# saurabh260918/Graph-Attention-Network-GATv2-

Measured on AMD Instinct MI355X. Metric: edges/sec (fwd+bwd, 2-layer 8-head GATv2), higher is better.
Workload: dtype f32; 1 GPU; products-shape synthetic power-law graph, 2450000 nodes / 61900000 edges / 100 feat / 47 classes, 2-layer GATv2 heads [8, 8] outdims [8, 8], fp32; launch=eager, parallelism=single GPU, generator=device (csrc/gat_synth.hip), bit-for-bit synth.py

## Files before the change

### graph-attention-network-gatv2-_amd/csrc/gat_dense_kernels.hip

```cpp
#include "gat_internal.h"

#include <algorithm>

#include <cstdlib>

namespace gat {
namespace {

struct MapIdentity {
    __device__ __forceinline__ int64_t operator()(int64_t idx) const { return idx; }
};
struct MapGradW {
    int32_t HD, F, c_base;
    __device__ __forceinline__ int64_t operator()(int64_t idx) const {
        const int32_t c = c_base + (int32_t)idx / F, f = (int32_t)idx % F;
        return (int64_t)(c % HD) * 2 * F + (c / HD) * F + f;
    }
};
template <class MAP>
__global__ __launch_bounds__(1024) void reduce_slabs_kernel(const float* __restrict__ slabs, int32_t nslabs,
                                                           int64_t width, float* __restrict__ out, MAP map) {
    __shared__ float part[16][64];
    const int q = threadIdx.x & 63, sl = threadIdx.x >> 6;
    const int64_t idx = (int64_t)blockIdx.x * 64 + q;
// ... 195 lines not shown
                const int lab_r = A.labels[n0 + r];
                s_dz[r * ldz + c] = lab_r >= 0 ? yt[q] - (c == lab_r ? 1.0f : 0.0f) : 0.0f;
                r += dqC; c += drC;
                if (c >= C) { c -= C; ++r; }
            }
        }
        for (int q = threadIdx.x; q < rows_here * DL; q += 256) s_hl[q] = A.HL[n0 * DL + q];
        __syncthreads();
        {
            int r = threadIdx.x / DL, d = threadIdx.x % DL;
            for (int q = threadIdx.x; q < rows_here * DL; q += 256) {
                float sum = 0.f;
                for (int c = 0; c < C; ++c) sum += s_wo[c * DL + d] * s_dz[r * ldz + c];
                s_gh[q] = sum;
                r += dqD; d += drD;
                if (d >= DL) { d -= DL; ++r; }
            }
        }
#pragma unroll
        for (int p = 0; p < 8; ++p) {
            const int t = threadIdx.x + p * 256;
            if (p < per_thread && t < C * DL) {
                const int c = t / DL, d = t % DL;
                float acc = wacc[p];
                for (int r = 0; r < rows_here; ++r) acc += s_dz[r * ldz + c] * s_hl[r * DL + d];
                wacc[p] = acc;
            }
        }
        __syncthreads();
        if (A.gh_out != nullptr)
            for (int q = threadIdx.x; q < rows_here * DL; q += 256) A.gh_out[(n0 + q / DL) * (A.gh_stride ? A.gh_stride : DL) + q % DL] = s_gh[q];
        if (A.g != nullptr) {
            const float* hp = A.hpre + n0 * hd;
            float* gt = A.g + n0 * hd;
            int r = threadIdx.x / hd, x = threadIdx.x % hd;
            for (int q = threadIdx.x; q < rows_here * hd; q += 256) {
                const int d = x % DL;
                const float hv = A.flat_index ? A.hpre[(n0 + r) * DL + d] : hp[q];
                gt[q] = s_gh[r * DL + d] * (hv > 0.f ? 1.0f : A.slope) * inv_heads;
                r += dqH; x += drH;
                if (x >= hd) { x -= hd; ++r; }
            }
        }
        __syncthreads();
    }
#pragma unroll
    for (int p = 0; p < 8; ++p) {
        const int t = threadIdx.x + p * 256;
        if (p < per_thread && t < C * DL) A.partial[(int64_t)blockIdx.x * C * DL + t] = wacc[p];
    }
}

template <int DL>
__global__ __launch_bounds__(256) void head_backward2_kernel(HeadBwdArgs A, int32_t ldz) {
    constexpr int NB = 128;
    extern __shared__ float lds[];
    const int C = A.C;
    float* s_wo = lds;
    float* s_dz = s_wo + C * DL;
    float* s_hl = s_dz + NB * ldz;
    for (int i = threadIdx.x; i < C * DL; i += 256) s_wo[i] = A.Wo[i];
    const int tid = threadIdx.x;
    const int t2 = tid - 128;
    const int wc = t2 >= 0 ? t2 % C : 0, whalf = t2 >= 0 ? t2 / C : 2;
    float wacc[DL];
#pragma unroll
    for (int d = 0; d < DL; ++d) wacc[d] = 0.f;
    const int64_t ntiles = (A.n_rows + NB - 1) / NB;
    const int dqC = 256 / C, drC = 256 % C;
    for (int64_t tile = blockIdx.x; tile < ntiles; tile += gridDim.x) {
        const int64_t n0 = tile * NB;
        const int rows_here = (int)((A.n_rows - n0 < NB) ? (A.n_rows - n0) : NB);
        __syncthreads();
        {
            const float* yt = A.y + n0 * C;
            int r = tid / C, c = tid % C;
            for (int q = tid; q < rows_here * C; q += 256) {
                const int lab_r = A.labels[n0 + r];
                s_dz[r * ldz + c] = lab_r >= 0 ? yt[q] - (c == lab_r ? 1.0f : 0.0f) : 0.0f;
                r += dqC; c += drC;
                if (c >= C) { c -= C; ++r; }
            }
        }
        for (int q = tid; q < rows_here * DL; q += 256) s_hl[q] = A.HL[n0 * DL + q];
        __syncthreads();
        if (tid < 128) {
            if (tid < rows_here) {
                float acc[DL];
#pragma unroll
                for (int d = 0; d < DL; ++d) acc[d] = 0.f;
                const float* zr = s_dz + tid * ldz;
                for (int c = 0; c < C; ++c) {
                    const float z = zr[c];
#pragma unroll
                    for (int d = 0; d < DL; ++d) acc[d] += s_wo[c * DL + d] * z;
                }
                float* out = A.gh_out + (n0 + tid) * (A.gh_stride ? A.gh_stride : DL);
#pragma unroll
                for (int d = 0; d < DL; ++d) out[d] = acc[d];
            }
        } else if (whalf < 2) {
            const int r0 = whalf * 64, r1 = (r0 + 64 < rows_here) ? r0 + 64 : rows_here;
            for (int r = r0; r < r1; ++r) {
                const float z = s_dz[r * ldz + wc];
#pragma unroll
                for (int d = 0; d < DL; ++d) wacc[d] += z * s_hl[r * DL + d];
            }
        }
    }
    __syncthreads();
    float* s_tmp = s_dz;
    if (whalf < 2) {
#pragma unroll
        for (int d = 0; d < DL; ++d) s_tmp[(whalf * C + wc) * DL + d] = wacc[d];
    }
    __syncthreads();
    for (int i = tid; i < C * DL; i += 256) A.partial[(int64_t)blockIdx.x * C * DL + i] = s_tmp[i] + s_tmp[C * DL + i];
}

template <int DL>
__global__ __launch_bounds__(256) void head_step_kernel(HeadArgs F, HeadBwdArgs A, int32_t ldz) {
    constexpr int NB = 128;
    extern __shared__ float lds[];
    const int C = A.C;
    float* s_wo = lds;
    float* s_dz = s_wo + C * DL;
    float* s_hl = s_dz + NB * ldz;
    __shared__ double s_loss[2];
    __shared__ int32_t s_corr[2];
    for (int i = threadIdx.x; i < C * DL; i += 256) s_wo[i] = A.Wo[i];
    const int tid = threadIdx.x;
    const int t2 = tid - 128;
    const int wc = t2 >= 0 ? t2 % C : 0, whalf = t2 >= 0 ? t2 / C : 2;
    float wacc[DL];
#pragma unroll
    for (int d = 0; d < DL; ++d) wacc[d] = 0.f;
    double loss_acc = 0.0;
    int corr_acc = 0;
    const int64_t ntiles = (A.n_rows + NB - 1) / NB;
    for (int64_t tile = blockIdx.x; tile < ntiles; tile += gridDim.x) {
        const int64_t n0 = tile * NB;
        const int rows_here = (int)((A.n_rows - n0 < NB) ? (A.n_rows - n0) : NB);
        __syncthreads();
        if (tid < rows_here) {
            const int64_t n = n0 + tid;
            float x[DL];
#pragma unroll
            for (int j = 0; j < DL; ++j) { x[j] = A.HL[n * DL + j]; s_hl[tid * DL + j] = x[j]; }
            float* zr = s_dz + tid * ldz;
            float mv = -INFINITY;
            for (int c = 0; c < C; ++c) {
                float acc = 0.f;
#pragma unroll
                for (int j = 0; j < DL; ++j) acc += s_wo[c * DL + j] * x[j];
                zr[c] = acc;
                mv = fmaxf(mv, acc);
            }
            float sum = 0.f;
            for (int c = 0; c < C; ++c) { const float ev = __builtin_amdgcn_exp2f((zr[c] - mv) * 1.4426950408889634f); zr[c] = ev; sum += ev; }
            const double rden = 1.0 / ((double)sum + 1e-8);
            const int lab = A.labels[n];
            float best = -1.f; int pred = 0; float plab = 0.f;
            for (int c = 0; c < C; ++c) {
                const float yv = (float)((double)zr[c] * rden);
                if (c == 0 || yv > best) { best = yv; pred = c; }
                if (c == lab) plab = yv;
                zr[c] = lab >= 0 ? yv - (c == lab ? 1.0f : 0.0f) : 0.0f;
            }
            loss_acc += lab >= 0 ? (double)(-logf(fmaxf(plab, 1e-12f))) : 0.0;
            corr_acc += (lab >= 0 && pred == lab) ? 1 : 0;
        }
        __syncthreads();
        if (tid < 128) {
            if (tid < rows_here) {
                float acc[DL];
#pragma unroll
                for (int d = 0; d < DL; ++d) acc[d] = 0.f;
                const float* zr = s_dz + tid * ldz;
                for (int c = 0; c < C; ++c) {
                    const float z = zr[c];
#pragma unroll
                    for (int d = 0; d < DL; ++d) acc[d] += s_wo[c * DL + d] * z;
                }
                if (A.gh_out != nullptr) {
                    float* out = A.gh_out + (n0 + tid) * (A.gh_stride ? A.gh_stride : DL);
#pragma unroll
                    for (int d = 0; d < DL; ++d) out[d] = acc[d];
                }
            }
        } else if (whalf < 2) {
            const int r0 = whalf * 64, r1 = (r0 + 64 < rows_here) ? r0 + 64 : rows_here;
            for (int r = r0; r < r1; ++r) {
                const float z = s_dz[r * ldz + wc];
#pragma unroll
                for (int d = 0; d < DL; ++d) wacc[d] += z * s_hl[r * DL + d];
            }
        }
    }
    __syncthreads();
    float* s_tmp = s_dz;
    if (whalf < 2) {
#pragma unroll
        for (int d = 0; d < DL; ++d) s_tmp[(whalf * C + wc) * DL + d] = wacc[d];
    }
    for (int off = 32; off > 0; off >>= 1) {
        loss_acc += __shfl_down(loss_acc, off);
        corr_acc += __shfl_down(corr_acc, off);
    }
    if (tid < 128 && (tid & 63) == 0) { s_loss[tid >> 6] = loss_acc; s_corr[tid >> 6] = corr_acc; }
    __syncthreads();
    for (int i = tid; i < C * DL; i += 256) A.partial[(int64_t)blockIdx.x * C * DL + i] = s_tmp[i] + s_tmp[C * DL + i];
    if (tid == 0) {
        F.loss_partial[blockIdx.x] = s_loss[0] + s_loss[1];
        F.correct_partial[blockIdx.x] = s_corr[0] + s_corr[1];
    }
}

__global__ __launch_bounds__(256) void sgd_kernel(float* p, const float* g, float lr, int64_t n) {
    const int64_t i = (int64_t)blockIdx.x * blockDim.x + threadIdx.x;
    if (i < n) p[i] -= lr * g[i];
}
__global__ __launch_bounds__(256) void adam_kernel(float* p, const float* g, float* m, float* v, float lr,
                                                  int64_t n, float b1, float b2, float eps, int32_t t) {
    const int64_t i = (int64_t)blockIdx.x * blockDim.x + threadIdx.x;
    if (i < n) {
        const float gi = g[i];
        const float mi = b1 * m[i] + (1.0f - b1) * gi;
        const float vi = b2 * v[i] + (1.0f - b2) * (gi * gi);
        m[i] = mi; v[i] = vi;
        const float mh = mi / (1.0f - powf(b1, (float)t));
        const float vh = vi / (1.0f - powf(b2, (float)t));
        p[i] -= lr * mh / (sqrtf(vh) + eps);
    }
}
__global__ __launch_bounds__(1024) void sumsq_kernel(const float* __restrict__ g, int64_t n, float* out) {
    __shared__ float part[16];
    float s = 0.f;
    for (int64_t i = threadIdx.x; i < n; i += blockDim.x) s += g[i] * g[i];
    for (int off = 32; off > 0; off >>= 1) s += __shfl_down(s, off);
    if ((threadIdx.x & 63) == 0) part[threadIdx.x >> 6] = s;
    __syncthreads();
    if (threadIdx.x == 0) {
        float t = 0.f;
        for (int w = 0; w < 16; ++w) t += part[w];
        *out = t;
    }
}
__global__ __launch_bounds__(256) void clip_scale_kernel(float* g, int64_t n, const float* sumsq, float thresh) {
    const float norm = sqrtf(*sumsq);
    float scale = 1.0f;
    if (norm > thresh) scale = thresh / (norm + 1e-9f);
    if (!(scale < 1.0f)) return;
    const int64_t i = (int64_t)blockIdx.x * blockDim.x + threadIdx.x;
    if (i < n) g[i] *= scale;
}

template <int V>
__global__ __launch_bounds__(256) void res_backward_kernel(ResBwdArgs A, int32_t LPR, int32_t rpb) {
    __shared__ float red[256 * 4];
    const int HD = A.H * A.D;
    const int t = threadIdx.x;
    const int r_in = t / LPR, cl = t % LPR;
    const float inv_heads = 1.0f / (float)A.H;
    for (int base = 0; base < HD; base += LPR * V) {
        const int c0 = base + cl * V;
        const bool active = r_in < rpb && c0 < HD;
        float sum[V];
// ... 270 lines not shown
    return 0;
}

int launch_reduce_partials_add(const float* partial, int32_t nblocks, int64_t width, float* out, hipStream_t s) {
    if (width <= 0) return 0;
    if (reduce_batch_push(partial, nblocks, width, out, 0, 0, 0)) return 0;
    hipLaunchKernelGGL((reduce_slabs_kernel<MapIdentity>), dim3((unsigned)((width + 63) / 64)), dim3(1024), 0, s,
                       partial, nblocks, width, out, MapIdentity{});
    GAT_HIP(hipGetLastError());
    return 0;
}

static int head_tile(int32_t C, int32_t DL, int32_t extra_per_row, int32_t* NB, int32_t* ldz) {
    const int l = (C % 2 == 0) ? C + 1 : C;
    int64_t budget = 60 * 1024 / 4 - (int64_t)C * DL;
    int nb = 256;
    while (nb >= 32 && (int64_t)nb * (l + extra_per_row) > budget) nb >>= 1;
    if (nb < 32) return fail(GAT_E_UNSUPPORTED, "output head: num_classes*D_last too large for the LDS tile");
    *NB = nb; *ldz = l;
    return 0;
}
int head_blocks(int64_t n_rows) {
    static const int per = [] { const char* e = choice_env("GAT_HEAD_NODES"); const int v = e ? atoi(e) : 0; return v == 256 ? 256 : 128; }();
    const int64_t b = (n_rows + per - 1) / per;
    return (int)(b < 1 ? 1 : (b > 2048 ? 2048 : b));
}
int launch_head_forward(const HeadArgs& a, hipStream_t s) {
    int32_t NB, ldz;
    const int dlp = a.DL <= 8 ? 8 : (a.DL <= 16 ? 16 : (a.DL <= 32 ? 32 : (a.DL <= 64 ? 64 : 0)));
    GAT_TRY(head_tile(a.C, dlp ? dlp : a.DL, 0, &NB, &ldz));
    int blocks = head_blocks(a.n_rows);
    const size_t lds = ((size_t)a.C * (dlp ? dlp : a.DL) + (size_t)NB * ldz) * sizeof(float);
    {
        const void* fn = dlp == 8 ? (const void*)head_forward_kernel<8> : dlp == 16 ? (const void*)head_forward_kernel<16>
                       : dlp == 32 ? (const void*)head_forward_kernel<32> : dlp == 64 ? (const void*)head_forward_kernel<64>
                                                                                      : (const void*)head_forward_kernel<0>;
        const int64_t res = resident_blocks(fn, lds);
        if (res < blocks) blocks = (int)res;
    }
    switch (dlp) {
        case 8: hipLaunchKernelGGL(head_forward_kernel<8>, dim3(blocks), dim3(256), lds, s, a, NB, ldz); break;
        case 16: hipLaunchKernelGGL(head_forward_kernel<16>, dim3(blocks), dim3(256), lds, s, a, NB, ldz); break;
        case 32: hipLaunchKernelGGL(head_forward_kernel<32>, dim3(blocks), dim3(256), lds, s, a, NB, ldz); break;
        case 64: hipLaunchKernelGGL(head_forward_kernel<64>, dim3(blocks), dim3(256), lds, s, a, NB, ldz); break;
        default: hipLaunchKernelGGL(head_forward_kernel<0>, dim3(blocks), dim3(256), lds, s, a, NB, ldz); break;
    }
    GAT_HIP(hipGetLastError());
    hipLaunchKernelGGL(head_finalize_kernel, dim3(1), dim3(64), 0, s, a.loss_partial, a.correct_partial, blocks,
                       a.loss_out, a.correct_out);
    GAT_HIP(hipGetLastError());
    return 0;
}
bool head_step_supported(const HeadBwdArgs& b) {
    return b.g == nullptr && b.gh_out != nullptr && b.C <= 64 && (b.DL == 4 || b.DL == 8 || b.DL == 16);
}
int launch_head_step(const HeadArgs& f, const HeadBwdArgs& b, hipStream_t s) {
    HeadBwdArgs probe = b;
    if (probe.gh_out == nullptr) probe.gh_out = reinterpret_cast<float*>(1);
    if (!head_step_supported(probe)) return fail(GAT_E_UNSUPPORTED, "head_step: shape outside the fused kernel");
    const int ldz = (b.C % 2 == 0) ? b.C + 1 : b.C;
    const size_t lds = ((size_t)b.C * b.DL + (size_t)128 * (ldz + b.DL)) * sizeof(float);
    int blocks = std::min(head_blocks(b.n_rows), head_bwd_blocks(b.n_rows, b.C, b.DL));
    const void* fn = b.DL == 4 ? (const void*)head_step_kernel<4> : b.DL == 8 ? (const void*)head_step_kernel<8>
                                                                                : (const void*)head_step_kernel<16>;
    const int64_t res = resident_blocks(fn, lds);
    if (res < blocks) blocks = (int)res;
    if (blocks < 1) blocks = 1;
    if (b.DL == 4) hipLaunchKernelGGL(head_step_kernel<4>, dim3(blocks), dim3(256), lds, s, f, b, ldz);
    else if (b.DL == 8) hipLaunchKernelGGL(head_step_kernel<8>, dim3(blocks), dim3(256), lds, s, f, b, ldz);
    else hipLaunchKernelGGL(head_step_kernel<16>, dim3(blocks), dim3(256), lds, s, f, b, ldz);
    GAT_HIP(hipGetLastError());
    if (!reduce_batch_finalize(f.loss_partial, f.correct_partial, blocks, f.loss_out, f.correct_out)) {
        hipLaunchKernelGGL(head_finalize_kernel, dim3(1), dim3(64), 0, s, f.loss_partial, f.correct_partial, blocks,
                           f.loss_out, f.correct_out);
        GAT_HIP(hipGetLastError());
    }
    return launch_reduce_partials_add(b.partial, blocks, (int64_t)b.C * b.DL, b.gradWo, s);
}
int launch_pack_result(const float* loss, const int32_t* correct, float* dst3, hipStream_t s) {
    hipLaunchKernelGGL(pack_result_kernel, dim3(1), dim3(64), 0, s, loss, correct, dst3);
    GAT_HIP(hipGetLastError());
    return 0;
}
int head_bwd_blocks(int64_t n_rows, int32_t C, int32_t DL) {
    (void)C; (void)DL;
    const int64_t b = (n_rows + 127) / 128;
    return (int)(b < 1 ? 1 : (b > 1024 ? 1024 : b));
}
int launch_head_backward(const HeadBwdArgs& a, hipStream_t s) {
    if (a.g == nullptr && a.gh_out != nullptr && a.C <= 64 && (a.DL == 4 || a.DL == 8 || a.DL == 16)) {
        const int ldz = (a.C % 2 == 0) ? a.C + 1 : a.C;
        const size_t lds = ((size_t)a.C * a.DL + (size_t)128 * (ldz + a.DL)) * sizeof(float);
        int blocks = (int)std::min<int64_t>((a.n_rows + 127) / 128, 1024);
        const void* fn = a.DL == 4 ? (const void*)head_backward2_kernel<4> : a.DL == 8 ? (const void*)head_backward2_kernel<8>
                                                                                        : (const void*)head_backward2_kernel<16>;
        const int64_t res = resident_blocks(fn, lds);
        if (res < blocks) blocks = (int)res;
        if (blocks < 1) blocks = 1;
        if (a.DL == 4) hipLaunchKernelGGL(head_backward2_kernel<4>, dim3(blocks), dim3(256), lds, s, a, ldz);
        else if (a.DL == 8) hipLaunchKernelGGL(head_backward2_kernel<8>, dim3(blocks), dim3(256), lds, s, a, ldz);
        else hipLaunchKernelGGL(head_backward2_kernel<16>, dim3(blocks), dim3(256), lds, s, a, ldz);
        GAT_HIP(hipGetLastError());
        return launch_reduce_partials_add(a.partial, blocks, (int64_t)a.C * a.DL, a.gradWo, s);
    }
    int32_t NB, ldz;
    GAT_TRY(head_tile(a.C, a.DL, 2 * a.DL, &NB, &ldz));
    const int per_thread = (a.C * a.DL + 255) / 256;
    if (per_thread > 8) return fail(GAT_E_UNSUPPORTED, "output head: num_classes*D_last > 2048");
    int blocks = head_bwd_blocks(a.n_rows, a.C, a.DL);
    const size_t lds = ((size_t)a.C * a.DL + (size_t)NB * (ldz + 2 * a.DL)) * sizeof(float);
    {
        const int64_t res = resident_blocks((const void*)head_backward_kernel, lds);
        if (res < blocks) blocks = (int)res;
    }
    hipLaunchKernelGGL(head_backward_kernel, dim3(blocks), dim3(256), lds, s, a, NB, ldz, per_thread);
    GAT_HIP(hipGetLastError());
    return launch_reduce_partials_add(a.partial, blocks, (int64_t)a.C * a.DL, a.gradWo, s);
}

__global__ __launch_bounds__(256) void apply_mask_kernel(const int32_t* __restrict__ labels, const uint8_t* __restrict__ mask,
                                                         int32_t* __restrict__ eff, int64_t n) {
    const int64_t stride = (int64_t)gridDim.x * blockDim.x;
    for (int64_t i = (int64_t)blockIdx.x * blockDim.x + threadIdx.x; i < n; i += stride)
        eff[i] = (mask == nullptr || mask[i]) ? labels[i] : ~labels[i];
}
int launch_apply_mask(const int32_t* labels, const uint8_t* mask, int32_t* eff, int64_t n, hipStream_t s) {
    if (n <= 0) return 0;
    hipLaunchKernelGGL(apply_mask_kernel, dim3((unsigned)std::min<int64_t>((n + 255) / 256, 4096)), dim3(256), 0, s, labels, mask, eff, n);
    GAT_HIP(hipGetLastError());
    return 0;
}
__global__ __launch_bounds__(256) void eval_mask_kernel(const float* __restrict__ y, const int32_t* __restrict__ labels,
                                                        const uint8_t* __restrict__ mask, int64_t n, int32_t C,
                                                        double* __restrict__ part_loss, int32_t* __restrict__ part_cnt) {
    __shared__ double s_l[256];
    __shared__ int32_t s_c[256], s_n[256];
    double l = 0.0; int32_t cr = 0, nn = 0;
    for (int64_t i = (int64_t)blockIdx.x * 256 + threadIdx.x; i < n; i += (int64_t)gridDim.x * 256) {
        if (!mask[i]) continue;
        const float* yr = y + i * C;
        const int lab = labels[i];
        float best = -1.f; int pred = 0;
        for (int c = 0; c < C; ++c) if (c == 0 || yr[c] > best) { best = yr[c]; pred = c; }
        l += (double)(-logf(fmaxf(yr[lab], 1e-12f)));
        cr += pred == lab; ++nn;
    }
    s_l[threadIdx.x] = l; s_c[threadIdx.x] = cr; s_n[threadIdx.x] = nn;
    __syncthreads();
    for (int off = 128; off > 0; off >>= 1) {
        if (threadIdx.x < off) { s_l[threadIdx.x] += s_l[threadIdx.x + off]; s_c[threadIdx.x] += s_c[threadIdx.x + off]; s_n[threadIdx.x] += s_n[threadIdx.x + off]; }
        __syncthreads();
    }
    if (threadIdx.x == 0) { part_loss[blockIdx.x] = s_l[0]; part_cnt[2 * blockIdx.x] = s_c[0]; part_cnt[2 * blockIdx.x + 1] = s_n[0]; }
}
int launch_eval_mask(const float* y, const int32_t* labels, const uint8_t* mask, int64_t n, int32_t C, double* part_loss,
                     int32_t* part_cnt, int32_t blocks, hipStream_t s) {
// ... 50 lines not shown
```

### graph-attention-network-gatv2-_amd/csrc/gat_gemm_kernels.hip

```cpp
#include "gat_internal.h"

#include <cstdlib>
#include <map>
#include <mutex>
#include <utility>

namespace gat {
namespace {

typedef float v16f __attribute__((ext_vector_type(16)));

struct ASrcRows {
    const float* X; int32_t ld;
    __device__ __forceinline__ float4 load4(int64_t i, int k) const {
        return *reinterpret_cast<const float4*>(X + i * ld + k);
    }
    __device__ __forceinline__ float load1(int64_t i, int k) const { return X[i * ld + k]; }
};
struct ASrcGcat {
    const float* gPL; const float* gPR; int32_t HD;
    __device__ __forceinline__ float4 load4(int64_t i, int k) const {
        return k < HD ? *reinterpret_cast<const float4*>(gPL + i * HD + k)
                      : *reinterpret_cast<const float4*>(gPR + i * HD + (k - HD));
    }
// ... 42 lines not shown
                PL[i * HD + j] = v;
            }
        } else {
            PR[i * HD + (j - HD)] = v;
        }
    }
};
struct EpiGradX {
    static constexpr bool kTwoPhase = true;
    float* out; const float* hpre_prev; int32_t ld; float slope;
    __device__ __forceinline__ float pre(int64_t i, int j) const { return hpre_prev[i * ld + j]; }
    __device__ __forceinline__ void apply(int64_t i, int j, float v, float hv) const {
        out[i * ld + j] = v * (hv > 0.f ? 1.0f : slope);
    }
    __device__ __forceinline__ void operator()(int64_t i, int j, float v) const { apply(i, j, v, pre(i, j)); }
};

struct EpiStore {
    static constexpr bool kTwoPhase = false;
    float* out; int32_t ld;
    __device__ __forceinline__ float pre(int64_t, int) const { return 0.f; }
    __device__ __forceinline__ void apply(int64_t i, int j, float v, float) const { out[i * ld + j] = v; }
    __device__ __forceinline__ void operator()(int64_t i, int j, float v) const { out[i * ld + j] = v; }
};

struct EpiAccum {
    static constexpr bool kTwoPhase = true;
    float* out; int32_t ld;
    __device__ __forceinline__ float pre(int64_t i, int j) const { return out[i * ld + j]; }
    __device__ __forceinline__ void apply(int64_t i, int j, float v, float old) const { out[i * ld + j] = old + v; }
    __device__ __forceinline__ void operator()(int64_t i, int j, float v) const { apply(i, j, v, pre(i, j)); }
};

constexpr int kKC = 128;

}

int64_t resident_blocks(const void* fn, size_t dyn_lds, int threads) {
    static std::mutex mu;
    static std::map<std::pair<const void*, size_t>, int64_t> cache;
    std::lock_guard<std::mutex> lock(mu);
    const auto key = std::make_pair(fn, dyn_lds);
    auto it = cache.find(key);
    if (it != cache.end()) return it->second;
    int per_cu = 0, dev = 0, cus = 256;
    if (hipOccupancyMaxActiveBlocksPerMultiprocessor(&per_cu, fn, threads, dyn_lds) != hipSuccess || per_cu < 1) per_cu = 1;
    if (per_cu > 8) per_cu = 8;
    (void)hipGetDevice(&dev);
    (void)hipDeviceGetAttribute(&cus, hipDeviceAttributeMultiprocessorCount, dev);
    (void)hipGetLastError();
    return cache[key] = (int64_t)per_cu * (cus > 0 ? cus : 256);
}

static void allow_big_lds(const void* fn) {
    static std::mutex mu;
    static std::map<std::pair<const void*, int>, bool> done;
    int dev = 0;
    (void)hipGetDevice(&dev);
    std::lock_guard<std::mutex> lock(mu);
    bool& d = done[std::make_pair(fn, dev)];
    if (!d) { (void)hipFuncSetAttribute(fn, hipFuncAttributeMaxDynamicSharedMemorySize, 160 * 1024); (void)hipGetLastError(); d = true; }
}

namespace {

template <int NT, bool VEC4, class AS, class BS, class EP>
__global__ __launch_bounds__(256) void rowgemm_kernel(AS as, BS bs, EP ep, int64_t M, int32_t N, int32_t K,
                                                      int32_t kc_lds) {
    constexpr int NW = NT * 32;
    extern __shared__ float Bsh[];
    const int lane = threadIdx.x & 63, wave = threadIdx.x >> 6;
    const int li = lane & 31, half = lane >> 5;
    const int n0 = blockIdx.y * NW;
    const int64_t ntiles = (M + 127) / 128;
    bool b_loaded = false;
    for (int64_t tile = blockIdx.x; tile < ntiles; tile += gridDim.x) {
        const int64_t row = tile * 128 + wave * 32 + li;
        const bool rvalid = row < M;
        v16f acc[NT];
#pragma unroll
        for (int nt = 0; nt < NT; ++nt)
#pragma unroll
            for (int r = 0; r < 16; ++r) acc[nt][r] = 0.f;
        for (int k0 = 0; k0 < K; k0 += kKC) {
            const int kc = (K - k0 < kKC) ? (K - k0) : kKC;
            const int kc8 = (kc + 7) & ~7;
            if (K > kKC || !b_loaded) {
                __syncthreads();
                if constexpr (BS::kAlongK) {
                    for (int idx = threadIdx.x; idx < kc8 * NW; idx += 256) {
                        const int kk = idx % kc8, j = idx / kc8;
                        Bsh[kk * NW + j] = (kk < kc && n0 + j < N) ? bs.at(k0 + kk, n0 + j) : 0.f;
                    }
                } else {
                    for (int idx = threadIdx.x; idx < kc8 * NW; idx += 256) {
                        const int kk = idx / NW, j = idx % NW;
                        Bsh[kk * NW + j] = (kk < kc && n0 + j < N) ? bs.at(k0 + kk, n0 + j) : 0.f;
                    }
                }
                b_loaded = true;
                __syncthreads();
            }
            float4 af[kKC / 8];
#pragma unroll
            for (int st = 0; st < kKC / 8; ++st) {
                const int kk = st * 8 + 4 * half;
                af[st] = make_float4(0.f, 0.f, 0.f, 0.f);
// ... 965 lines not shown
```

### graph-attention-network-gatv2-_amd/csrc/gat_internal.h

```cpp
#pragma once
#include <hip/hip_runtime.h>
#include <cstdint>
#include <cstdio>
#include <string>
#include <vector>

#include "gatv2_abi.h"

namespace gat {

constexpr int kWave = 64;

void set_error(const std::string& msg);
int fail(int code, const std::string& msg);
const char* choice_env(const char* name);

#define GAT_HIP(expr)                                                                     \
    do {                                                                                  \
        hipError_t e__ = (expr);                                                          \
        if (e__ != hipSuccess)                                                            \
            return ::gat::fail((int)e__, std::string(#expr) + ": " + hipGetErrorString(e__)); \
    } while (0)

#define GAT_TRY(expr)                 \
// ... 204 lines not shown
int launch_gpl_pull(const SourceIndex& ix, const PullArgs& p, hipStream_t s);

int launch_csr_to_coo(const int32_t* row_ptr, const int32_t* col_idx, int32_t* src, int32_t* dst,
                      int64_t n_rows, int64_t n_edges, int64_t table_row0, hipStream_t s);

struct Comm {
    int world = 1, rank = 0;
    virtual ~Comm();
    virtual int all_gather(float* table, int64_t slice, hipStream_t s) = 0;
    virtual int all_gather_part(float* table, int64_t slice, int64_t off, int64_t cnt, hipStream_t s) = 0;
    virtual int reduce_scatter(float* table, int64_t slice, hipStream_t s) = 0;
    virtual int reduce_scatter_bf16(float* table, int64_t slice, hipStream_t s) = 0;
    virtual int all_reduce(float* buf, int64_t n, hipStream_t s) = 0;
    virtual int exchange_rows(const float* sendbuf, const int64_t* cnt_send, float* recvbuf, const int64_t* cnt_recv, int64_t rf, hipStream_t s) = 0;
};
struct HaloPlan {
    int world = 0, rank = 0;
    int64_t max_rows = 0;
    std::vector<int64_t> need_cnt, send_cnt;
    int64_t n_need = 0, n_send = 0, buf_rows = 0;
    int32_t* need_rows = nullptr;
    int32_t* send_rows = nullptr;
    int32_t *arr_ptr = nullptr, *arr_split = nullptr, *arr_pos = nullptr;
    float *sendbuf = nullptr, *recvbuf = nullptr;
    double referenced_fraction = 1.0;
};
int halo_build(Comm* comm, const int32_t* d_col_idx, int64_t n_edges, int64_t n_table, int32_t hd_max, HaloPlan* out, hipStream_t s);
int halo_forward(Comm* comm, const HaloPlan& h, float* table, int64_t rf, hipStream_t s);
int halo_backward(Comm* comm, const HaloPlan& h, float* gPL, int64_t rf, hipStream_t s);
void halo_free(HaloPlan* h);
int comm_unique_id(void* id_out);
int comm_create_rccl(int world, int rank, const void* id_bytes, Comm** out);
int comm_create_host(int world, int rank, const char* shm_name, int64_t bytes_per_rank, Comm** out);

int launch_pack_result(const float* loss, const int32_t* correct, float* dst3, hipStream_t s);
struct ReduceJob { const float* slabs; float* out; int64_t width; int32_t nslabs, HD, F, c_base, block0; };
struct ReduceBatch {
    ReduceJob jobs[8]; int32_t n, blocks;
    const float* loss; const int32_t* correct; float* dst3; float* dst3_host;
    const double* fin_loss; const int32_t* fin_corr; int32_t fin_n; float* fin_loss_out; int32_t* fin_corr_out;
};
void reduce_batch_begin();
void reduce_batch_abort();
void reduce_batch_pack(const float* loss, const int32_t* correct, float* dst3, float* dst3_host);
bool reduce_batch_finalize(const double* loss_partial, const int32_t* correct_partial, int32_t nblocks, float* loss_out, int32_t* correct_out);
int reduce_batch_flush(hipStream_t s);
int launch_reduce_partials_add(const float* partial, int32_t nblocks, int64_t width, float* out,
                               hipStream_t s);

int launch_reduce_gradw(const float* slabs, int32_t ksplit, int32_t HD, int32_t F, int32_t c_base, int32_t M,
                        float* gradW, hipStream_t s);

int64_t resident_blocks(const void* fn, size_t dyn_lds, int threads = 256);

int launch_transpose_eh_to_he(const float* src_eh, float* dst_he, int64_t E, int32_t H, hipStream_t s);
int launch_transpose_he_to_eh(const float* src_he, float* dst_eh, int64_t E, int32_t H, hipStream_t s);
int launch_transpose_nh_to_hn(const float* src_nh, float* dst_hn, int64_t N, int32_t H, hipStream_t s);

enum : int32_t { kPartBoth = 0, kPartLeft = 1, kPartRight = 2 };
int64_t project_scratch_floats(int64_t n_rows, int32_t F, int32_t HD, int32_t part);
int launch_project(const float* X, const float* W, float* PL_rows, float* PR, int64_t n_rows,
                   int32_t F, int32_t HD, int32_t part, bool pl_bf16, float* scratch, int64_t scratch_floats, hipStream_t s, int32_t ldx = 0);
int64_t grad_w_scratch_floats(int64_t n_rows, int32_t F, int32_t HD);
int launch_grad_w(const float* gPL_rows, const float* gPR, const float* X, float* gradW,
                  float* scratch, int64_t n_rows, int32_t F, int32_t HD, int32_t part, hipStream_t s, int32_t ldx = 0);
int launch_grad_x(const float* gPL_rows, const float* gPR, const float* W, const float* hpre_prev,
                  float* gprev, int64_t n_rows, int32_t F, int32_t HD, float slope, hipStream_t s);

int launch_project_res(const float* X, const float* Wres, float* R, int64_t n_rows, int32_t F, int32_t HD, hipStream_t s, int32_t ldx = 0);
int launch_grad_wres(const float* G, const float* X, float* gradWres, float* scratch, int64_t n_rows, int32_t F, int32_t HD,
                     hipStream_t s, int32_t ldx = 0);
int launch_grad_x_res(const float* G, const float* Wres, float* gx, int64_t n_rows, int32_t F, int32_t HD, hipStream_t s);
struct ResBwdArgs {
    const float* hpre; const float* g; const float* gh; const float* res; const float* bias;
    float* G; float* agg; float* partial;
    int64_t n_rows;
    int32_t H, D, gh_stride, g_raw, blocks;
    float slope;
};
constexpr int kResPartialRows = 1024;
int res_backward_blocks(int64_t n_rows, int32_t HD);
int launch_res_backward(const ResBwdArgs& a, hipStream_t s);

struct NormBwdArgs {
    ResBwdArgs r;
    const float* gamma; const float* beta;
    float* part_gamma; float* part_beta;
    float eps;
};
int norm_backward_blocks(int64_t n_rows, int32_t HD);
int launch_norm_backward(const NormBwdArgs& a, hipStream_t s);

struct HeadArgs {
    const float* Wo;
    const float* HL;
    const int32_t* labels;
    float* y;
    double* loss_partial;
    int32_t* correct_partial;
    float* loss_out;
    int32_t* correct_out;
    int64_t n_rows;
    int32_t C, DL;
};
int head_blocks(int64_t n_rows);
int launch_head_forward(const HeadArgs& a, hipStream_t s);
// ... 77 lines not shown
```

Before: 2.970 billion edges/s.

## Restructure output-head kernels with 256-row tiles, register softmax, and virtual-block partials

Reworks the fused head step and head backward kernels. Tiles grow to 256 rows and all 256 threads now do both the per-row gradient and the Wo-gradient accumulation. Partials are written per fixed virtual block (capped at 1024) instead of per launched block, so the reduction width no longer depends on occupancy. In the step kernel, logits and softmax stay in registers with the class count padded to a compile-time size, HL rows are prefetched with float4 loads for the next tile, and gradient outputs are stored as float4. The cost is more LDS per block (it may need the big-LDS opt-in), more frequent flush barriers, an alignment requirement for the fused path, and more template instantiations.

```diff
diff --git a/graph-attention-network-gatv2-_amd/csrc/gat_dense_kernels.hip b/graph-attention-network-gatv2-_amd/csrc/gat_dense_kernels.hip
--- a/graph-attention-network-gatv2-_amd/csrc/gat_dense_kernels.hip
+++ b/graph-attention-network-gatv2-_amd/csrc/gat_dense_kernels.hip
@@ -271,23 +271,57 @@
 }
 
 template <int DL>
-__global__ __launch_bounds__(256) void head_backward2_kernel(HeadBwdArgs A, int32_t ldz) {
-    constexpr int NB = 128;
-    extern __shared__ float lds[];
+__device__ __forceinline__ void head_wo_tile(const float* s_dz, int ldz, const float* s_hl, int wc, int r0, int r1, float (&wacc)[DL]) {
+    for (int r = r0; r < r1; ++r) {
+        const float zv = s_dz[r * ldz + wc];
+        float h[DL];
+#pragma unroll
+        for (int v = 0; v < DL / 4; ++v) {
+            const float4 q = reinterpret_cast<const float4*>(s_hl + r * DL)[v];
+            h[4 * v] = q.x; h[4 * v + 1] = q.y; h[4 * v + 2] = q.z; h[4 * v + 3] = q.w;
+        }
+#pragma unroll
+        for (int d = 0; d < DL; ++d) wacc[d] = __builtin_fmaf(zv, h[d], wacc[d]);
+    }
+}
+template <int DL>
+__device__ __forceinline__ void head_wo_flush(float* s_tmp, int C, int G, bool owner, float (&wacc)[DL], float* __restrict__ out) {
+    const int tid = threadIdx.x;
+    __syncthreads();
+    if (owner) {
+#pragma unroll
+        for (int d = 0; d < DL; ++d) { s_tmp[tid * DL + d] = wacc[d]; wacc[d] = 0.f; }
+    }
+    __syncthreads();
+    for (int i = tid; i < C * DL; i += 256) {
+        float t = s_tmp[i];
+        for (int g = 1; g < G; ++g) t += s_tmp[g * C * DL + i];
+        out[i] = t;
+    }
+}
+__device__ __forceinline__ void head_next_tile(int64_t ntiles, int VB, int64_t& vb, int64_t& tile) {
+    tile += VB;
+    if (tile >= ntiles) { vb += gridDim.x; tile = vb; }
+}
+
+template <int DL>
+__global__ __launch_bounds__(256) void head_backward2_kernel(HeadBwdArgs A, int32_t ldz, int32_t G, int32_t RPG, int32_t VB) {
+    constexpr int NB = 256;
+    extern __shared__ float4 lds_waves[];
     const int C = A.C;
-    float* s_wo = lds;
+    float* s_hl = reinterpret_cast<float*>(lds_waves);
+    float* s_wo = s_hl + NB * DL;
     float* s_dz = s_wo + C * DL;
-    float* s_hl = s_dz + NB * ldz;
-    for (int i = threadIdx.x; i < C * DL; i += 256) s_wo[i] = A.Wo[i];
     const int tid = threadIdx.x;
-    const int t2 = tid - 128;
-    const int wc = t2 >= 0 ? t2 % C : 0, whalf = t2 >= 0 ? t2 / C : 2;
+    for (int i = tid; i < C * DL; i += 256) s_wo[i] = A.Wo[i];
+    const int wc = tid % C, wg = tid / C;
     float wacc[DL];
 #pragma unroll
     for (int d = 0; d < DL; ++d) wacc[d] = 0.f;
     const int64_t ntiles = (A.n_rows + NB - 1) / NB;
     const int dqC = 256 / C, drC = 256 % C;
-    for (int64_t tile = blockIdx.x; tile < ntiles; tile += gridDim.x) {
+    int64_t vb = blockIdx.x, tile = vb;
+    while (vb < VB) {
         const int64_t n0 = tile * NB;
         const int rows_here = (int)((A.n_rows - n0 < NB) ? (A.n_rows - n0) : NB);
         __syncthreads();
@@ -303,135 +337,143 @@
         }
         for (int q = tid; q < rows_here * DL; q += 256) s_hl[q] = A.HL[n0 * DL + q];
         __syncthreads();
-        if (tid < 128) {
-            if (tid < rows_here) {
-                float acc[DL];
-#pragma unroll
-                for (int d = 0; d < DL; ++d) acc[d] = 0.f;
-                const float* zr = s_dz + tid * ldz;
-                for (int c = 0; c < C; ++c) {
-                    const float z = zr[c];
-#pragma unroll
-                    for (int d = 0; d < DL; ++d) acc[d] += s_wo[c * DL + d] * z;
-                }
-                float* out = A.gh_out + (n0 + tid) * (A.gh_stride ? A.gh_stride : DL);
-#pragma unroll
-                for (int d = 0; d < DL; ++d) out[d] = acc[d];
-            }
-        } else if (whalf < 2) {
-            const int r0 = whalf * 64, r1 = (r0 + 64 < rows_here) ? r0 + 64 : rows_here;
-            for (int r = r0; r < r1; ++r) {
-                const float z = s_dz[r * ldz + wc];
-#pragma unroll
-                for (int d = 0; d < DL; ++d) wacc[d] += z * s_hl[r * DL + d];
-            }
-        }
-    }
-    __syncthreads();
-    float* s_tmp = s_dz;
-    if (whalf < 2) {
-#pragma unroll
-        for (int d = 0; d < DL; ++d) s_tmp[(whalf * C + wc) * DL + d] = wacc[d];
-    }
-    __syncthreads();
-    for (int i = tid; i < C * DL; i += 256) A.partial[(int64_t)blockIdx.x * C * DL + i] = s_tmp[i] + s_tmp[C * DL + i];
+        if (tid < rows_here) {
+            float acc[DL];
+#pragma unroll
+            for (int d = 0; d < DL; ++d) acc[d] = 0.f;
+            const float* zr = s_dz + tid * ldz;
+            for (int c = 0; c < C; ++c) {
+                const float z = zr[c];
+#pragma unroll
+                for (int d = 0; d < DL; ++d) acc[d] = __builtin_fmaf(s_wo[c * DL + d], z, acc[d]);
+            }
+            float* out = A.gh_out + (n0 + tid) * (A.gh_stride ? A.gh_stride : DL);
+#pragma unroll
+            for (int d = 0; d < DL; ++d) out[d] = acc[d];
+        }
+        if (wg < G) head_wo_tile<DL>(s_dz, ldz, s_hl, wc, wg * RPG, (wg * RPG + RPG < rows_here) ? wg * RPG + RPG : rows_here, wacc);
+        const int64_t done = vb;
+        head_next_tile(ntiles, VB, vb, tile);
+        if (vb != done) head_wo_flush<DL>(s_dz, C, G, wg < G, wacc, A.partial + done * C * DL);
+    }
 }
 
 template <int DL>
-__global__ __launch_bounds__(256) void head_step_kernel(HeadArgs F, HeadBwdArgs A, int32_t ldz) {
-    constexpr int NB = 128;
-    extern __shared__ float lds[];
+__device__ __forceinline__ float head_logit(const float* w, const float* x, float z0) {
+    constexpr int NF = DL == 16 ? 4 : 0;
+    float acc = z0;
+#pragma unroll
+    for (int j = 0; j < NF; ++j) acc = __builtin_fmaf(w[j], x[j], acc);
+    {
+#pragma clang fp contract(off)
+#pragma unroll
+        for (int j = NF; j < DL; ++j) acc = acc + w[j] * x[j];
+    }
+    return acc;
+}
+template <int V>
+__device__ __forceinline__ void head_row_load(const float* p, float4 (&x)[V]) {
+#pragma unroll
+    for (int v = 0; v < V; ++v) x[v] = reinterpret_cast<const float4*>(p)[v];
+}
+
+template <int DL, int CP>
+__global__ __launch_bounds__(256) void head_step_kernel(HeadArgs F, HeadBwdArgs A, int32_t G, int32_t RPG, int32_t VB) {
+    constexpr int NB = 256, V = DL / 4, ldz = CP + 1;
+    extern __shared__ float4 lds_waves[];
     const int C = A.C;
-    float* s_wo = lds;
-    float* s_dz = s_wo + C * DL;
-    float* s_hl = s_dz + NB * ldz;
-    __shared__ double s_loss[2];
-    __shared__ int32_t s_corr[2];
-    for (int i = threadIdx.x; i < C * DL; i += 256) s_wo[i] = A.Wo[i];
+    float* s_hl = reinterpret_cast<float*>(lds_waves);
+    float* s_wo = s_hl + NB * DL;
+    float* s_z0 = s_wo + CP * DL;
+    float* s_dz = s_z0 + CP;
+    __shared__ double s_loss[4];
+    __shared__ int32_t s_corr[4];
     const int tid = threadIdx.x;
-    const int t2 = tid - 128;
-    const int wc = t2 >= 0 ? t2 % C : 0, whalf = t2 >= 0 ? t2 / C : 2;
+    for (int i = tid; i < CP * DL; i += 256) s_wo[i] = i < C * DL ? A.Wo[i] : 0.f;
+    if (tid < CP) s_z0[tid] = tid < C ? 0.f : -INFINITY;
+    const int wc = tid % C, wg = tid / C;
     float wacc[DL];
 #pragma unroll
     for (int d = 0; d < DL; ++d) wacc[d] = 0.f;
     double loss_acc = 0.0;
     int corr_acc = 0;
     const int64_t ntiles = (A.n_rows + NB - 1) / NB;
-    for (int64_t tile = blockIdx.x; tile < ntiles; tile += gridDim.x) {
+    const int gstride = A.gh_stride ? A.gh_stride : DL;
+    float4 xn[V] = {};
+    int labn = -1;
+    int64_t vb = blockIdx.x, tile = vb;
+    if (vb < VB && tile * NB + tid < A.n_rows) {
+        head_row_load<V>(A.HL + (tile * NB + tid) * DL, xn);
+        labn = A.labels[tile * NB + tid];
+    }
+    while (vb < VB) {
         const int64_t n0 = tile * NB;
         const int rows_here = (int)((A.n_rows - n0 < NB) ? (A.n_rows - n0) : NB);
+        float x[DL];
+#pragma unroll
+        for (int v = 0; v < V; ++v) { x[4 * v] = xn[v].x; x[4 * v + 1] = xn[v].y; x[4 * v + 2] = xn[v].z; x[4 * v + 3] = xn[v].w; }
+        const int lab = labn;
+        const int64_t done = vb;
+        head_next_tile(ntiles, VB, vb, tile);
+        if (vb < VB && tile * NB + tid < A.n_rows) {
+            head_row_load<V>(A.HL + (tile * NB + tid) * DL, xn);
+            labn = A.labels[tile * NB + tid];
+        }
         __syncthreads();
         if (tid < rows_here) {
-            const int64_t n = n0 + tid;
-            float x[DL];
-#pragma unroll
-            for (int j = 0; j < DL; ++j) { x[j] = A.HL[n * DL + j]; s_hl[tid * DL + j] = x[j]; }
+#pragma unroll
+            for (int v = 0; v < V; ++v) reinterpret_cast<float4*>(s_hl + tid * DL)[v] = make_float4(x[4 * v], x[4 * v + 1], x[4 * v + 2], x[4 * v + 3]);
+            float z[CP];
+            float mv = -INFINITY;
+#pragma unroll
+            for (int c = 0; c < CP; ++c) {
+                const float acc = head_logit<DL>(s_wo + c * DL, x, s_z0[c]);
+                z[c] = acc;
+                mv = fmaxf(mv, acc);
+            }
+            float sum = 0.f;
+#pragma unroll
+            for (int c = 0; c < CP; ++c) { const float ev = __builtin_amdgcn_exp2f((z[c] - mv) * 1.4426950408889634f); z[c] = ev; sum += ev; }
+            const double rden = 1.0 / ((double)sum + 1e-8);
+            float best = -1.f; int pred = 0; float plab = 0.f;
             float* zr = s_dz + tid * ldz;
-            float mv = -INFINITY;
-            for (int c = 0; c < C; ++c) {
-                float acc = 0.f;
-#pragma unroll
-                for (int j = 0; j < DL; ++j) acc += s_wo[c * DL + j] * x[j];
-                zr[c] = acc;
-                mv = fmaxf(mv, acc);
-            }
-            float sum = 0.f;
-            for (int c = 0; c < C; ++c) { const float ev = __builtin_amdgcn_exp2f((zr[c] - mv) * 1.4426950408889634f); zr[c] = ev; sum += ev; }
-            const double rden = 1.0 / ((double)sum + 1e-8);
-            const int lab = A.labels[n];
-            float best = -1.f; int pred = 0; float plab = 0.f;
-            for (int c = 0; c < C; ++c) {
-                const float yv = (float)((double)zr[c] * rden);
+#pragma unroll
+            for (int c = 0; c < CP; ++c) {
+                const float yv = (float)((double)z[c] * rden);
                 if (c == 0 || yv > best) { best = yv; pred = c; }
                 if (c == lab) plab = yv;
-                zr[c] = lab >= 0 ? yv - (c == lab ? 1.0f : 0.0f) : 0.0f;
+                z[c] = lab >= 0 ? yv - (c == lab ? 1.0f : 0.0f) : 0.0f;
+                zr[c] = z[c];
             }
             loss_acc += lab >= 0 ? (double)(-logf(fmaxf(plab, 1e-12f))) : 0.0;
             corr_acc += (lab >= 0 && pred == lab) ? 1 : 0;
+            if (A.gh_out != nullptr) {
+                float acc[DL];
+#pragma unroll
+                for (int d = 0; d < DL; ++d) acc[d] = 0.f;
+#pragma unroll
+                for (int c = 0; c < CP; ++c) {
+#pragma unroll
+                    for (int d = 0; d < DL; ++d) acc[d] = __builtin_fmaf(s_wo[c * DL + d], z[c], acc[d]);
+                }
+                float4* out = reinterpret_cast<float4*>(A.gh_out + (n0 + tid) * gstride);
+#pragma unroll
+                for (int v = 0; v < V; ++v) out[v] = make_float4(acc[4 * v], acc[4 * v + 1], acc[4 * v + 2], acc[4 * v + 3]);
+            }
         }
         __syncthreads();
-        if (tid < 128) {
-            if (tid < rows_here) {
-                float acc[DL];
-#pragma unroll
-                for (int d = 0; d < DL; ++d) acc[d] = 0.f;
-                const float* zr = s_dz + tid * ldz;
-                for (int c = 0; c < C; ++c) {
-                    const float z = zr[c];
-#pragma unroll
-                    for (int d = 0; d < DL; ++d) acc[d] += s_wo[c * DL + d] * z;
-                }
-                if (A.gh_out != nullptr) {
-                    float* out = A.gh_out + (n0 + tid) * (A.gh_stride ? A.gh_stride : DL);
-#pragma unroll
-                    for (int d = 0; d < DL; ++d) out[d] = acc[d];
-                }
-            }
-        } else if (whalf < 2) {
-            const int r0 = whalf * 64, r1 = (r0 + 64 < rows_here) ? r0 + 64 : rows_here;
-            for (int r = r0; r < r1; ++r) {
-                const float z = s_dz[r * ldz + wc];
-#pragma unroll
-                for (int d = 0; d < DL; ++d) wacc[d] += z * s_hl[r * DL + d];
-            }
-        }
-    }
-    __syncthreads();
-    float* s_tmp = s_dz;
-    if (whalf < 2) {
-#pragma unroll
-        for (int d = 0; d < DL; ++d) s_tmp[(whalf * C + wc) * DL + d] = wacc[d];
+        if (wg < G) head_wo_tile<DL>(s_dz, ldz, s_hl, wc, wg * RPG, (wg * RPG + RPG < rows_here) ? wg * RPG + RPG : rows_here, wacc);
+        if (vb != done) head_wo_flush<DL>(s_dz, C, G, wg < G, wacc, A.partial + done * C * DL);
     }
     for (int off = 32; off > 0; off >>= 1) {
         loss_acc += __shfl_down(loss_acc, off);
         corr_acc += __shfl_down(corr_acc, off);
     }
-    if (tid < 128 && (tid & 63) == 0) { s_loss[tid >> 6] = loss_acc; s_corr[tid >> 6] = corr_acc; }
+    if ((tid & 63) == 0) { s_loss[tid >> 6] = loss_acc; s_corr[tid >> 6] = corr_acc; }
     __syncthreads();
-    for (int i = tid; i < C * DL; i += 256) A.partial[(int64_t)blockIdx.x * C * DL + i] = s_tmp[i] + s_tmp[C * DL + i];
     if (tid == 0) {
-        F.loss_partial[blockIdx.x] = s_loss[0] + s_loss[1];
-        F.correct_partial[blockIdx.x] = s_corr[0] + s_corr[1];
+        F.loss_partial[blockIdx.x] = (s_loss[0] + s_loss[1]) + (s_loss[2] + s_loss[3]);
+        F.correct_partial[blockIdx.x] = (s_corr[0] + s_corr[1]) + (s_corr[2] + s_corr[3]);
     }
 }
 
@@ -808,30 +850,52 @@
     return 0;
 }
 bool head_step_supported(const HeadBwdArgs& b) {
-    return b.g == nullptr && b.gh_out != nullptr && b.C <= 64 && (b.DL == 4 || b.DL == 8 || b.DL == 16);
+    const bool vec16 = ((reinterpret_cast<uintptr_t>(b.HL) | reinterpret_cast<uintptr_t>(b.gh_out)) & 15) == 0 && b.gh_stride % 4 == 0;
+    return b.g == nullptr && b.gh_out != nullptr && b.C <= 64 && (b.DL == 4 || b.DL == 8 || b.DL == 16) && vec16;
+}
+struct HeadTree { int32_t VB, G, RPG; };
+static HeadTree head_tree(int64_t n_rows, int32_t C) {
+    const int64_t tiles = (n_rows + 255) / 256;
+    HeadTree t;
+    t.VB = (int32_t)(tiles < 1 ? 1 : (tiles > 1024 ? 1024 : tiles));
+    t.G = 256 / C;
+    t.RPG = (256 + t.G - 1) / t.G;
+    return t;
+}
+template <int DL, int CP>
+static int launch_head_step_cp(const HeadArgs& f, const HeadBwdArgs& b, const HeadTree& t, int* blocks_out, hipStream_t s) {
+    const size_t lds = ((size_t)256 * DL + (size_t)CP * DL + CP + (size_t)256 * std::max(CP + 1, DL)) * sizeof(float);
+    const void* fn = (const void*)head_step_kernel<DL, CP>;
+    if (lds > 64 * 1024) allow_big_lds(fn);
+    int64_t blocks = std::min<int64_t>(t.VB, resident_blocks(fn, lds));
+    if (blocks < 1) blocks = 1;
+    hipLaunchKernelGGL((head_step_kernel<DL, CP>), dim3((unsigned)blocks), dim3(256), lds, s, f, b, t.G, t.RPG, t.VB);
+    GAT_HIP(hipGetLastError());
+    *blocks_out = (int)blocks;
+    return 0;
+}
+template <int DL>
+static int launch_head_step_dl(const HeadArgs& f, const HeadBwdArgs& b, const HeadTree& t, int* blocks_out, hipStream_t s) {
+    if (b.C <= 16) return launch_head_step_cp<DL, 16>(f, b, t, blocks_out, s);
+    if (b.C <= 32) return launch_head_step_cp<DL, 32>(f, b, t, blocks_out, s);
+    if (b.C <= 48) return launch_head_step_cp<DL, 48>(f, b, t, blocks_out, s);
+    return launch_head_step_cp<DL, 64>(f, b, t, blocks_out, s);
 }
 int launch_head_step(const HeadArgs& f, const HeadBwdArgs& b, hipStream_t s) {
     HeadBwdArgs probe = b;
-    if (probe.gh_out == nullptr) probe.gh_out = reinterpret_cast<float*>(1);
+    if (probe.gh_out == nullptr) probe.gh_out = const_cast<float*>(b.HL);
     if (!head_step_supported(probe)) return fail(GAT_E_UNSUPPORTED, "head_step: shape outside the fused kernel");
-    const int ldz = (b.C % 2 == 0) ? b.C + 1 : b.C;
-    const size_t lds = ((size_t)b.C * b.DL + (size_t)128 * (ldz + b.DL)) * sizeof(float);
-    int blocks = std::min(head_blocks(b.n_rows), head_bwd_blocks(b.n_rows, b.C, b.DL));
-    const void* fn = b.DL == 4 ? (const void*)head_step_kernel<4> : b.DL == 8 ? (const void*)head_step_kernel<8>
-                                                                                : (const void*)head_step_kernel<16>;
-    const int64_t res = resident_blocks(fn, lds);
-    if (res < blocks) blocks = (int)res;
-    if (blocks < 1) blocks = 1;
-    if (b.DL == 4) hipLaunchKernelGGL(head_step_kernel<4>, dim3(blocks), dim3(256), lds, s, f, b, ldz);
-    else if (b.DL == 8) hipLaunchKernelGGL(head_step_kernel<8>, dim3(blocks), dim3(256), lds, s, f, b, ldz);
-    else hipLaunchKernelGGL(head_step_kernel<16>, dim3(blocks), dim3(256), lds, s, f, b, ldz);
-    GAT_HIP(hipGetLastError());
+    const HeadTree t = head_tree(b.n_rows, b.C);
+    int blocks = 0;
+    if (b.DL == 4) GAT_TRY((launch_head_step_dl<4>(f, b, t, &blocks, s)));
+    else if (b.DL == 8) GAT_TRY((launch_head_step_dl<8>(f, b, t, &blocks, s)));
+    else GAT_TRY((launch_head_step_dl<16>(f, b, t, &blocks, s)));
     if (!reduce_batch_finalize(f.loss_partial, f.correct_partial, blocks, f.loss_out, f.correct_out)) {
         hipLaunchKernelGGL(head_finalize_kernel, dim3(1), dim3(64), 0, s, f.loss_partial, f.correct_partial, blocks,
                            f.loss_out, f.correct_out);
         GAT_HIP(hipGetLastError());
     }
-    return launch_reduce_partials_add(b.partial, blocks, (int64_t)b.C * b.DL, b.gradWo, s);
+    return launch_reduce_partials_add(b.partial, t.VB, (int64_t)b.C * b.DL, b.gradWo, s);
 }
 int launch_pack_result(const float* loss, const int32_t* correct, float* dst3, hipStream_t s) {
     hipLaunchKernelGGL(pack_result_kernel, dim3(1), dim3(64), 0, s, loss, correct, dst3);
@@ -845,19 +909,19 @@
 }
 int launch_head_backward(const HeadBwdArgs& a, hipStream_t s) {
     if (a.g == nullptr && a.gh_out != nullptr && a.C <= 64 && (a.DL == 4 || a.DL == 8 || a.DL == 16)) {
+        const HeadTree t = head_tree(a.n_rows, a.C);
         const int ldz = (a.C % 2 == 0) ? a.C + 1 : a.C;
-        const size_t lds = ((size_t)a.C * a.DL + (size_t)128 * (ldz + a.DL)) * sizeof(float);
-        int blocks = (int)std::min<int64_t>((a.n_rows + 127) / 128, 1024);
+        const size_t lds = ((size_t)256 * a.DL + (size_t)a.C * a.DL + (size_t)256 * std::max(ldz, a.DL)) * sizeof(float);
         const void* fn = a.DL == 4 ? (const void*)head_backward2_kernel<4> : a.DL == 8 ? (const void*)head_backward2_kernel<8>
                                                                                         : (const void*)head_backward2_kernel<16>;
-        const int64_t res = resident_blocks(fn, lds);
-        if (res < blocks) blocks = (int)res;
+        if (lds > 64 * 1024) allow_big_lds(fn);
+        int blocks = (int)std::min<int64_t>(t.VB, resident_blocks(fn, lds));
         if (blocks < 1) blocks = 1;
-        if (a.DL == 4) hipLaunchKernelGGL(head_backward2_kernel<4>, dim3(blocks), dim3(256), lds, s, a, ldz);
-        else if (a.DL == 8) hipLaunchKernelGGL(head_backward2_kernel<8>, dim3(blocks), dim3(256), lds, s, a, ldz);
-        else hipLaunchKernelGGL(head_backward2_kernel<16>, dim3(blocks), dim3(256), lds, s, a, ldz);
+        if (a.DL == 4) hipLaunchKernelGGL(head_backward2_kernel<4>, dim3(blocks), dim3(256), lds, s, a, ldz, t.G, t.RPG, t.VB);
+        else if (a.DL == 8) hipLaunchKernelGGL(head_backward2_kernel<8>, dim3(blocks), dim3(256), lds, s, a, ldz, t.G, t.RPG, t.VB);
+        else hipLaunchKernelGGL(head_backward2_kernel<16>, dim3(blocks), dim3(256), lds, s, a, ldz, t.G, t.RPG, t.VB);
         GAT_HIP(hipGetLastError());
-        return launch_reduce_partials_add(a.partial, blocks, (int64_t)a.C * a.DL, a.gradWo, s);
+        return launch_reduce_partials_add(a.partial, t.VB, (int64_t)a.C * a.DL, a.gradWo, s);
     }
     int32_t NB, ldz;
     GAT_TRY(head_tile(a.C, a.DL, 2 * a.DL, &NB, &ldz));
diff --git a/graph-attention-network-gatv2-_amd/csrc/gat_gemm_kernels.hip b/graph-attention-network-gatv2-_amd/csrc/gat_gemm_kernels.hip
--- a/graph-attention-network-gatv2-_amd/csrc/gat_gemm_kernels.hip
+++ b/graph-attention-network-gatv2-_amd/csrc/gat_gemm_kernels.hip
@@ -118,7 +118,7 @@
     return cache[key] = (int64_t)per_cu * (cus > 0 ? cus : 256);
 }
 
-static void allow_big_lds(const void* fn) {
+void allow_big_lds(const void* fn) {
     static std::mutex mu;
     static std::map<std::pair<const void*, int>, bool> done;
     int dev = 0;
diff --git a/graph-attention-network-gatv2-_amd/csrc/gat_internal.h b/graph-attention-network-gatv2-_amd/csrc/gat_internal.h
--- a/graph-attention-network-gatv2-_amd/csrc/gat_internal.h
+++ b/graph-attention-network-gatv2-_amd/csrc/gat_internal.h
@@ -280,6 +280,7 @@
                         float* gradW, hipStream_t s);
 
 int64_t resident_blocks(const void* fn, size_t dyn_lds, int threads = 256);
+void allow_big_lds(const void* fn);
 
 int launch_transpose_eh_to_he(const float* src_eh, float* dst_he, int64_t E, int32_t H, hipStream_t s);
 int launch_transpose_he_to_eh(const float* src_he, float* dst_eh, int64_t E, int32_t H, hipStream_t s);
```

Result: no change. 3.019 billion edges/s (median of 6 runs) (+1.7%).
